# mchitten/keto

Hardware: AMD Instinct MI355X
Metric: permission checks/sec (batched, whole node) + traversal HBM GB/s vs roofline (higher is better)
Workload: dtype u32 ids / u64 bitmasks (integer)

## Files before the change

### keto_amd/csrc/device_engine.hip

```cpp
#include <hip/hip_runtime.h>

#include <algorithm>
#include <atomic>
#include <chrono>
#include <cstring>
#include <functional>
#include <map>
#include <mutex>
#include <string>
#include <thread>
#include <type_traits>
#include <vector>

#include "core_index.hpp"
#include "device_util.hpp"
#include "labels.hpp"
#include "tier.hpp"
#include "ketogpu_internal.hpp"

using namespace ketogpu;
using namespace kdev;

namespace {

// ... 2215 lines not shown
    for (uint32_t step = 32; step; step >>= 1)
        if (step <= (uint32_t)E && pos + step <= (uint32_t)E && L[pos + step - 1] < x) pos += step;
    return pos;
}
template <int E>
__device__ __forceinline__ bool label_find_e(const uint32_t *L, uint32_t x) {
    const uint32_t pos = label_lower_e<E>(L, x);
    return pos < (uint32_t)E && L[pos] == x;
}

template <int E>
__device__ __forceinline__ bool label_block8(const uint32_t *L, uint32_t x) {
    static_assert(E % 8 == 4, "a head's inline entries");
    constexpr int NB = (E + 7) / 8;
    uint32_t blk = 0;
#pragma unroll
    for (int b = 0; b + 1 < NB; b++) blk += L[8 * b + 7] < x;
    const uint4 u = *reinterpret_cast<const uint4 *>(L + 8 * blk);
    const bool lo = min(min(u.x ^ x, u.y ^ x), min(u.z ^ x, u.w ^ x)) == 0;
    if constexpr (NB == 1) {
        return lo;
    } else {
        const uint4 v = *reinterpret_cast<const uint4 *>(L + 8 * blk + 4);
        const bool hi = min(min(v.x ^ x, v.y ^ x), min(v.z ^ x, v.w ^ x)) == 0;
        return lo | (hi & (blk != (uint32_t)(NB - 1)));
    }
}

template <int E, int H>
__device__ __forceinline__ bool label_lookup(const uint32_t *row, uint32_t x) {
    return label_block8<E>(row + kHeadFixed, x);
}

#ifndef KETO_LABEL_MEET
#define KETO_LABEL_MEET 0
#endif

template <int HS, int HP, bool TAIL = false>
__device__ __forceinline__ void label_unit(LabelShared<HS, HP> &sh, const LabelGraph &L, uint32_t r_lane,
                                           uint32_t t_lane, uint64_t *allowed, const uint64_t unit,
                                           const LabelRest &R, const LabelRest &F, unsigned long long *stats) {
    static_assert((HS == 8 || HS == 16 || HS == 32 || HS == 64) && (HP == 8 || HP == 16 || HP == 32 || HP == 64),
                  "heads of 8, 16, 32 or 64 words");
    constexpr int SW = HS / 4, PW = HP / 4;
    constexpr uint32_t CS = HS - kHeadFixed, CP = HP - kHeadFixed;
    const uint32_t lane = threadIdx.x & 63, q = lane >> 2, sub = lane & 3;
    const uint32_t r = (uint32_t)__shfl((int)r_lane, (int)q, 64), t = (uint32_t)__shfl((int)t_lane, (int)q, 64);
    const bool some = r != KETOGPU_NODE_NONE && t != KETOGPU_NODE_NONE;
    const bool valid = some && r < kDynBase;
    uint32_t sw[SW], pw[PW];
#pragma unroll
    for (int k = 0; k < SW; k++) sw[k] = 0xFFFFFFFFu;
#pragma unroll
    for (int k = 0; k < PW; k++) pw[k] = 0xFFFFFFFFu;
    if (valid) {
        label_head_load<SW>(L.S + (uint64_t)t * HS, sub, sw);
        label_head_load<PW>(L.P + (uint64_t)r * HP, sub, pw);
    }
    const uint32_t ns = label_word<SW, 0>(sw), np = label_word<PW, 0>(pw);
    const bool labelled = valid && ns != kNoLabel && np != kNoLabel;
    const uint64_t smask = (uint64_t)label_word<SW, 2>(sw) | (uint64_t)label_word<SW, 3>(sw) << 32;
    const uint64_t pmask = (uint64_t)label_word<PW, 2>(pw) | (uint64_t)label_word<PW, 3>(pw) << 32;
    uint32_t *Sl = sh.S + q * (HS + 4), *Pl = sh.P + q * (HP + 4);
    label_to_lds<SW>(Sl, sw, sub);
    label_to_lds<PW>(Pl, pw, sub);
    const uint32_t *Se = Sl + kHeadFixed, *Pe = Pl + kHeadFixed;
    const uint32_t shard = (uint32_t)(unit % kRestShards);
    {
        const bool rest = sub == 0 && some && !labelled;
        const uint32_t at = lds_append(rest, R.count + shard * kRestStride);
        if (rest) R.list[shard * R.cap + at] = (uint32_t)(unit * 16 + q);
// ... 5 lines not shown
#pragma unroll
    for (int k = 0; k < SW; k++) es += (k >= (int)kHeadFixed || s_body) && sw[k] < L.ni;
    es += (uint32_t)__builtin_amdgcn_update_dpp(0, (int)es, 0xB1, 0xf, 0xf, false);
    es += (uint32_t)__builtin_amdgcn_update_dpp(0, (int)es, 0x4E, 0xf, 0xf, false);
    if (!labelled) es = 0;
    const uint32_t ep = min(np, CP);
    {
        bool head = false, body = false;
#pragma unroll
        for (int k = 0; k < SW; k++) (k < (int)kHeadFixed ? head : body) |= sw[k] == r;
        hit |= labelled && r >= L.ni && (body | (head & s_body));
    }
    if (labelled && !hit) {
        if (KETO_LABEL_MEET == 2) {
            if (es <= ep)
                for (uint32_t k = sub; k < es && !hit; k += 4) hit = label_find_e<CP>(Pe, Se[k]);
            else
                for (uint32_t k = sub; k < ep && !hit; k += 4) hit = label_find_e<CS>(Se, Pe[k]);
        } else {
            if constexpr (HS == HP) {
                const bool ws = es <= ep;
                const uint32_t *W = ws ? Se : Pe, *O = ws ? Pl : Sl;
                const uint32_t e = ws ? es : ep;
                for (uint32_t k = sub; k < e && !hit; k += 4) hit = label_lookup<CP, HP>(O, W[k]);
            } else {
                if (es <= ep)
                    for (uint32_t k = sub; k < es && !hit; k += 4) hit = label_lookup<CP, HP>(Pl, Se[k]);
                else
                    for (uint32_t k = sub; k < ep && !hit; k += 4) hit = label_lookup<CS, HS>(Sl, Pe[k]);
            }
        }
    }
    bool tail = false;
    if constexpr (TAIL) {
        const uint64_t hq = __ballot(hit);
        bool tq = labelled && !((hq >> (lane & ~3u)) & 0xF) && np > CP && np <= 2 * CP && es > 0;
        uint32_t p_last = 0;
        if (tq) {
            const uint32_t s_end = Se[CS - 1];
            p_last = Pe[CP - 1];
            const bool s_whole = ns <= CS || s_end >= L.ni, raw_done = r < L.ni || ns <= CS || r <= s_end;
            tq = s_whole && raw_done && Se[es - 1] > p_last;
        }
        if (__ballot(tq)) {
            uint32_t k0 = 0;
#pragma unroll
            for (int k = 0; k < SW; k++) k0 += (k >= (int)kHeadFixed || s_body) && sw[k] <= p_last;
            k0 += (uint32_t)__builtin_amdgcn_update_dpp(0, (int)k0, 0xB1, 0xf, 0xf, false);
            k0 += (uint32_t)__builtin_amdgcn_update_dpp(0, (int)k0, 0x4E, 0xf, 0xf, false);
            constexpr int NT = (int)CP / 4, NL = (NT + 3) / 4;
            const uint4 *Tg = reinterpret_cast<const uint4 *>(L.P + (uint64_t)label_word<PW, 1>(pw) * 16) + CP / 4;
            uint4 tv[NL];
#pragma unroll
            for (int j = 0; j < NL; j++) {
                const uint32_t i = sub + 4 * j;
                tv[j] = make_uint4(0xFFFFFFFFu, 0xFFFFFFFFu, 0xFFFFFFFFu, 0xFFFFFFFFu);
                if (tq && i < (uint32_t)NT && CP + 4 * i < np) tv[j] = Tg[i];
            }
            wave_sync();
#pragma unroll
            for (int j = 0; j < NL; j++) {
                const uint32_t i = sub + 4 * j, w = CP + 4 * i;
                if (tq && i < (uint32_t)NT)
                    reinterpret_cast<uint4 *>(Pl)[1 + i] =
                        make_uint4(w < np ? tv[j].x : 0xFFFFFFFFu, w + 1 < np ? tv[j].y : 0xFFFFFFFFu,
                                   w + 2 < np ? tv[j].z : 0xFFFFFFFFu, w + 3 < np ? tv[j].w : 0xFFFFFFFFu);
            }
            wave_sync();
            if (tq)
                for (uint32_t k = k0 + sub; k < es && !hit; k += 4) hit = label_lookup<CP, HP>(Pl, Se[k]);
            tail = tq;
        }
    }
    {
        const uint64_t hb = __ballot(hit);
        const uint32_t os = label_word<SW, 1>(sw), op = label_word<PW, 1>(pw);
        bool full = false;
        if (sub == 0 && labelled && !tail && !((hb >> lane) & 0xF)) {
            const uint32_t s_end = Se[CS - 1];
            const bool s_whole = ns <= CS || s_end >= L.ni, p_whole = np <= CP;
            const uint32_t s_last = es ? Se[es - 1] : 0u, p_last = ep ? Pe[ep - 1] : 0u;
            const bool lm_done = es == 0 || np == 0 || (s_whole && (p_whole || s_last <= p_last)) ||
                                 (p_whole && p_last <= s_last);
            const bool raw_done = r < L.ni || ns <= CS || r <= s_end;
            full = !(lm_done && raw_done);
        }
        const uint32_t at = lds_append(full, F.count + shard * kRestStride);
        if (full) {
            uint4 *rec = F.rec + 2 * (shard * F.cap + at);
            rec[0] = make_uint4((uint32_t)(unit * 16 + q), r, t, ns);
            rec[1] = make_uint4(np, os, op, 0u);
        }
    }
    const uint64_t bits = __ballot(hit);
    uint32_t rows = 0, ent = 0;
    if (stats) {
        rows = wave_sum_all(labelled && sub == 0 ? 2u : 0u);
        ent = wave_sum_all(labelled && sub == 0 ? ns + np + kHeadFixed : 0u);
    }
    uint64_t x = bits | bits >> 1;
    x = (x | x >> 2) & 0x1111111111111111ull;
    x = (x | x >> 3) & 0x0303030303030303ull;
    x = (x | x >> 6) & 0x000F000F000F000Full;
    x = (x | x >> 12) & 0x000000FF000000FFull;
    x = (x | x >> 24) & 0xFFFFull;
    if (lane == 0) {
        reinterpret_cast<uint16_t *>(allowed)[unit] = (uint16_t)x;
        if (stats) {
            atomicAdd(&stat_slot(stats)[0], (unsigned long long)rows);
            atomicAdd(&stat_slot(stats)[2], (unsigned long long)ent);
        }
    }
}

__device__ __forceinline__ void label_clear_next(const LabelRest &R, const LabelRest &F) {
    if (blockIdx.x == 0 && threadIdx.x < 64) {
        R.next_count[threadIdx.x * kRestStride] = 0u;
        F.next_count[threadIdx.x * kRestStride] = 0u;
    }
}

template <int HS, int HP>
__global__ __launch_bounds__(64) void label_kernel(LabelGraph L, const uint32_t *roots, const uint32_t *targets,
                                                   uint64_t n, uint64_t *allowed, LabelRest R, LabelRest F,
                                                   unsigned long long *stats, uint64_t unit0) {
    __shared__ LabelShared<HS, HP> sh;
    if (unit0 == 0) label_clear_next(R, F);
    const uint64_t units = (n + 15) / 16;
    const uint64_t unit = unit0 + blockIdx.x;
    uint32_t r, t;
    bidi_load_rt<16>(unit, units, roots, targets, n, r, t);
    label_unit<HS, HP>(sh, L, r, t, allowed, unit, R, F, stats);
    if (unit + 1 == units && threadIdx.x == 0)
        for (uint64_t u = units; u < (units + 3) / 4 * 4; u++) reinterpret_cast<uint16_t *>(allowed)[u] = 0;
}

template <int HS, int HP>
__global__ __launch_bounds__(256) void label_host_kernel(DevGraph g, LabelGraph L, const uint32_t *hr,
                                                         const uint32_t *ht, uint32_t *dr, uint32_t *dt, uint64_t n,
                                                         uint64_t *allowed, LabelRest R, LabelRest F,
                                                         unsigned long long *stats, unsigned long long *first_bad) {
    __shared__ LabelShared<HS, HP> sh[4];
    __shared__ uint32_t rq[2][64];
    const uint32_t wave = threadIdx.x >> 6, lane = threadIdx.x & 63;
    label_clear_next(R, F);
    if (wave == 0) {
        uint32_t r[4], t[4];
        host_unit_requests<4>(g, hr, ht, dr, dt, n, first_bad, r, t);
        if (lane < 16)
#pragma unroll
            for (int k = 0; k < 4; k++) rq[0][16 * k + lane] = r[k], rq[1][16 * k + lane] = t[k];
    }
    __syncthreads();
    const uint64_t units = (n + 15) / 16;
    const uint64_t unit = (uint64_t)blockIdx.x * 4 + wave;
    if (unit >= units) return;
    const uint32_t rk = lane < 16 ? rq[0][16 * wave + lane] : KETOGPU_NODE_NONE;
    const uint32_t tk = lane < 16 ? rq[1][16 * wave + lane] : KETOGPU_NODE_NONE;
    label_unit<HS, HP>(sh[wave], L, rk, tk, allowed, unit, R, F, stats);
}

__device__ __forceinline__ void packed24_decode(uint32_t *raw, const uint64_t *src, uint64_t w0, uint64_t nwords,
                                                uint32_t lane, uint32_t &r, uint32_t &t) {
    if (lane < 48) {
        const uint64_t w = w0 + lane < nwords ? src[w0 + lane] : 0ull;
        *reinterpret_cast<uint2 *>(raw + 2 * lane) = make_uint2((uint32_t)w, (uint32_t)(w >> 32));
    }
    wave_sync();
    const uint32_t k = (3 * lane) >> 1;
    const uint64_t v = ((uint64_t)raw[k + 1] << 32 | raw[k]) >> ((lane & 1) * 16);
    r = (uint32_t)v & 0xFFFFFFu;
    t = (uint32_t)(v >> 24) & 0xFFFFFFu;
    if (r == 0xFFFFFFu) r = KETOGPU_NODE_NONE;
    if (t == 0xFFFFFFu) t = KETOGPU_NODE_NONE;
}

template <int HS, int HP>
__global__ __launch_bounds__(256) void label_host_packed_kernel(DevGraph g, LabelGraph L, const uint64_t *hp,
                                                                uint32_t *dr, uint32_t *dt, uint64_t n,
                                                                uint64_t *allowed, LabelRest R, LabelRest F,
                                                                unsigned long long *stats,
                                                                unsigned long long *first_bad) {
    __shared__ LabelShared<HS, HP> sh[4];
    __shared__ uint32_t rq[2][64];
    const uint32_t wave = threadIdx.x >> 6, lane = threadIdx.x & 63;
    label_clear_next(R, F);
    if (wave == 0) {
        uint32_t r, t;
        packed24_decode(&rq[0][0], hp, (uint64_t)blockIdx.x * 48, (6 * n + 7) / 8, lane, r, t);
        const uint64_t c = (uint64_t)blockIdx.x * 64 + lane;
        if (c < n) {
            if ((r != KETOGPU_NODE_NONE && r >= g.Nx) || (t != KETOGPU_NODE_NONE && t >= g.N)) {
                atomicMin(first_bad, (unsigned long long)c);
                r = t = KETOGPU_NODE_NONE;
            }
            dr[c] = r;
            dt[c] = t;
        } else {
            r = t = KETOGPU_NODE_NONE;
        }
        wave_sync();
        rq[0][lane] = r;
        rq[1][lane] = t;
    }
    __syncthreads();
    const uint64_t units = (n + 15) / 16;
    const uint64_t unit = (uint64_t)blockIdx.x * 4 + wave;
    if (unit >= units) return;
    const uint32_t rk = lane < 16 ? rq[0][16 * wave + lane] : KETOGPU_NODE_NONE;
    const uint32_t tk = lane < 16 ? rq[1][16 * wave + lane] : KETOGPU_NODE_NONE;
    label_unit<HS, HP>(sh[wave], L, rk, tk, allowed, unit, R, F, stats);
}

__host__ __device__ constexpr uint32_t full_stage(int HS, int HP) { return HS >= 64 || HP >= 64 ? 256u : 128u; }

template <int HS, int HP, uint32_t kStage, int kPre, int kFly>
__device__ __forceinline__ uint64_t label_dense_units(uint32_t *stage, const LabelGraph &L, uint64_t *allowed,
                                                      const LabelRest &F, const uint32_t c, const uint32_t first_u,
                                                      const uint32_t stride) {
    static_assert(kStage % 4 == 0, "16-byte aligned rows");
    const uint32_t lane = threadIdx.x, q = lane >> 2, sub = lane & 3;
    const uint32_t nu = (c + 15) / 16;
    const uint32_t incl = wave_incl_sum_u32(nu);
    const uint64_t units = (uint64_t)__builtin_amdgcn_readlane((int)incl, 63);
    uint32_t *row = stage + q * kStage;
    uint64_t ent = 0;
    for (uint64_t u = first_u; u < units; u += stride) {
        const uint32_t shard = (uint32_t)__builtin_ctzll(__ballot(incl > u));
        const uint32_t first = (uint32_t)__builtin_amdgcn_readlane((int)(incl - nu), (int)shard);
        const uint32_t cs = (uint32_t)__builtin_amdgcn_readlane((int)c, (int)shard);
        const uint64_t j = (u - first) * 16 + (lane & 15);
        uint4 r0 = make_uint4(KETOGPU_NODE_NONE, 0, 0, 0), r1 = make_uint4(0, 0, 0, 0);
        if (lane < 16 && j < cs) {
            const uint4 *rec = F.rec + 2 * (shard * F.cap + j);
            r0 = rec[0];
            r1 = rec[1];
        }
        const uint32_t idx = (uint32_t)__shfl((int)r0.x, (int)q, 64);
        const uint32_t rr = (uint32_t)__shfl((int)r0.y, (int)q, 64), tt = (uint32_t)__shfl((int)r0.z, (int)q, 64);
        const uint32_t ns = (uint32_t)__shfl((int)r0.w, (int)q, 64), np = (uint32_t)__shfl((int)r1.x, (int)q, 64);
        const uint32_t os = (uint32_t)__shfl((int)r1.y, (int)q, 64), op = (uint32_t)__shfl((int)r1.z, (int)q, 64);
        const bool valid = idx != KETOGPU_NODE_NONE;
        const bool s_over = ns > (uint32_t)(HS - kHeadFixed), p_over = np > (uint32_t)(HP - kHeadFixed);
        const uint32_t *Sg = s_over ? L.S + (uint64_t)os * 16 : L.S + (uint64_t)tt * HS + kHeadFixed;
        const uint32_t *Pg = p_over ? L.P + (uint64_t)op * 16 : L.P + (uint64_t)rr * HP + kHeadFixed;
        const bool walk_p = np <= ns;
        const uint32_t nw = walk_p ? np : ns, nl = walk_p ? ns : np;
        const uint32_t *Lg = walk_p ? Sg : Pg, *W = walk_p ? Pg : Sg;
        {
            constexpr int kSt = (kStage / 4 + 3) / 4;
            const bool st = valid && nl <= kStage;
#pragma unroll
            for (int k0 = 0; k0 < kSt; k0 += kFly) {
                uint4 v[kFly];
#pragma unroll
                for (int k = 0; k < kFly; k++) {
                    const uint32_t i = sub + 4 * (k0 + k);
                    v[k] = k0 + k < kSt && st && i * 4 < nl ? reinterpret_cast<const uint4 *>(Lg)[i]
                                                            : make_uint4(0u, 0u, 0u, 0u);
                }
#pragma unroll
                for (int k = 0; k < kFly; k++) {
                    const uint32_t i = sub + 4 * (k0 + k);
                    if (k0 + k < kSt && st && i * 4 < nl) reinterpret_cast<uint4 *>(row)[i] = v[k];
                }
            }
        }
        uint32_t wk[kPre];
#pragma unroll
        for (int i = 0; i < kPre; i++) {
            const uint32_t k = sub + 4 * i;
            wk[i] = valid && k < nw ? W[k] : 0u;
        }
        wave_sync();
        const uint32_t *O = nl <= kStage ? row : Lg;
        bool hit = false;
        if (valid) {
#pragma unroll
            for (int i = 0; i < kPre; i++)
                if (!hit && sub + 4 * i < nw) hit = label_find_n(O, nl, wk[i]);
            for (uint32_t k = sub + 4 * kPre; k < nw && !hit; k += 4) hit = label_find_n(O, nl, W[k]);
            if (sub == 0 && !hit && rr >= L.ni) hit = walk_p ? label_find_n(O, nl, rr) : label_find_n(W, nw, rr);
        }
        const uint64_t bits = __ballot(hit);
        if (valid && sub == 0) {
            if ((bits >> lane) & 0xF) atomicOr((unsigned long long *)&allowed[idx >> 6], 1ull << (idx & 63));
            ent += nl;
        }
        wave_sync();
    }
    return ent;
}

template <int HS, int HP>
__global__ __launch_bounds__(64) void label_full_kernel(LabelGraph L, uint64_t *allowed, LabelRest R, LabelRest F,
                                                        unsigned int *total_rest, unsigned int *total_full,
                                                        unsigned long long *stats, unsigned long long *mirror) {
    constexpr uint32_t kFullStage = full_stage(HS, HP);
    __shared__ alignas(16) uint32_t stage[16 * kFullStage];
    const uint32_t lane = threadIdx.x;
    const uint32_t c = F.count[lane * kRestStride];
    if (blockIdx.x == 0) {
        const uint32_t tr = wave_sum_all(R.count[lane * kRestStride]), tf = wave_sum_all(c);
        if (lane == 0) *total_rest = tr, *total_full = tf;
        if (mirror && lane < 12)
            mirror[lane] = lane == 8 ? (unsigned long long)tr : lane == 11 ? (unsigned long long)tf << 32 : 0ull;
    }
    const uint64_t ent =
        label_dense_units<HS, HP, kFullStage, 16, (int)kFullStage / 16>(stage, L, allowed, F, c, blockIdx.x, gridDim.x);
    const uint32_t e = wave_sum_all((uint32_t)ent);
    if (stats && lane == 0 && e) atomicAdd(&stat_slot(stats)[2], (unsigned long long)e);
}

template <int HS, int HP, bool TAIL>
__global__ __launch_bounds__(64) void label_carry_kernel(LabelGraph L, const uint32_t *roots, const uint32_t *targets,
                                                         uint64_t n, uint64_t *allowed, LabelRest R, LabelRest F,
                                                         LabelRest Fd, uint64_t *allowed_d, uint32_t D) {
    __shared__ LabelShared<HS, HP> sh;
    static_assert(sizeof(LabelShared<HS, HP>) == 64 * (HS + HP + 8), "the dense role's stage");
    if (blockIdx.x < D) {
        label_dense_units<HS, HP, HS + HP + 8, 4, 2>(reinterpret_cast<uint32_t *>(&sh), L, allowed_d, Fd,
                                                     Fd.count[threadIdx.x * kRestStride], blockIdx.x, D);
        return;
    }
    if (blockIdx.x == D) {
        R.next_count[threadIdx.x * kRestStride] = 0u;
        F.next_count[threadIdx.x * kRestStride] = 0u;
    }
    const uint64_t units = (n + 15) / 16;
    const uint64_t unit = blockIdx.x - D;
    uint32_t r, t;
    bidi_load_rt<16>(unit, units, roots, targets, n, r, t);
    label_unit<HS, HP, TAIL>(sh, L, r, t, allowed, unit, R, F, nullptr);
    if (unit + 1 == units && threadIdx.x == 0)
        for (uint64_t u = units; u < (units + 3) / 4 * 4; u++) reinterpret_cast<uint16_t *>(allowed)[u] = 0;
}

template <class SH>
__global__ __launch_bounds__(64) void label_rest_kernel(DevGraph g, const FRec *frec, const FRec *brec,
                                                        const uint32_t *roots, const uint32_t *targets,
                                                        uint64_t *allowed, LabelRest R, unsigned int *total,
                                                        uint32_t *out, unsigned int *out_count,
                                                        unsigned long long *stats) {
    __shared__ SH S;
    const uint32_t lane = threadIdx.x;
    const uint32_t c = R.count[lane * kRestStride];
    const uint32_t nu = (c + 15) / 16;
    const uint32_t incl = wave_incl_sum_u32(nu);
    const uint64_t units = (uint64_t)__builtin_amdgcn_readlane((int)incl, 63);
    const uint32_t listed = wave_sum_all(c);
    if (blockIdx.x == 0 && lane == 0) *total = listed;
    for (uint64_t u = blockIdx.x; u < units; u += gridDim.x) {
        const uint32_t shard = (uint32_t)__builtin_ctzll(__ballot(incl > u));
        const uint32_t first = (uint32_t)__builtin_amdgcn_readlane((int)(incl - nu), (int)shard);
        const uint32_t cs = (uint32_t)__builtin_amdgcn_readlane((int)c, (int)shard);
        const uint64_t j = (u - first) * 16 + lane;
        uint32_t idx = KETOGPU_NODE_NONE, r = KETOGPU_NODE_NONE, t = KETOGPU_NODE_NONE;
        if (lane < 16 && j < cs) {
            idx = R.list[shard * R.cap + j];
            r = roots[idx];
            t = targets[idx];
        }
        lite_unit<SH, false>(S, g, frec, brec, bidi_load_rows(g, r, t), allowed, u, out, out_count, stats, nullptr,
                             idx, true);
        __syncthreads();
    }
// ... 1437 lines not shown
    }();
    bool label_clean = false;
    bool lean_call = false;
    bool pipelined_req = false, queued = false;
    hipStream_t pipe_s[kPipe] = {};
    bool pipe_used[kPipe] = {};
    const ketogpu_queries *pipe_q[kPipe] = {};
    bool label_defer = [] {
        const char *e = getenv("KETOGPU_LABEL_DEFER");
        return !e || atoi(e) != 0;
    }();
    int done_mode = [] {
        const char *e = getenv("KETOGPU_LABEL_DONE_EVENT");
        return !e ? 2 : !strcmp(e, "record") ? 0 : !strcmp(e, "nofence") ? 1 : 2;
    }();
    struct PendingDense {
        bool on = false;
        ketogpu_queries *q = nullptr;
        uint64_t *allowed = nullptr;
        LabelRest R{}, F{};
    } pend[kPipe];
    bool carry_call = false;
    unsigned cur_pipe = 0;
    uint64_t pipe_epoch = 1;
    hipEvent_t order_ev = nullptr;
    hipStream_t pstream(unsigned k) const {
        if (k == cur_pipe) return stream;
        return k ? pipe_s[k] : pipe_s[cur_pipe];
    }
    bool label_tail = [] {
        const char *e = getenv("KETOGPU_LABEL_TAIL");
        return !e || atoi(e) != 0;
    }();
    uint64_t piped_full = 0;
    bool piped_full_known = false, flush_unread = false;
    void take_piped_full() {
        piped_full = ((const unsigned int *)(h_ctr + 24))[7];
        piped_full_known = true;
    }
    static unsigned grid_for(uint64_t full) { return (unsigned)std::min<uint64_t>(std::max<uint64_t>(full / 16 + 64, 64), 16384); }
    unsigned dense_grid() const { return grid_for(full_prev); }
    unsigned piped_grid() const { return grid_for(piped_full_known ? piped_full : full_prev); }
    bool flush_dense(unsigned k) {
        PendingDense p = pend[k];
        if (!p.on) return false;
        pend[k] = PendingDense{};
        label_dispatch([&](auto hs, auto hp) {
            KLAUNCH((label_full_kernel<decltype(hs)::value, decltype(hp)::value>), dim3(piped_grid()), dim3(64), 0,
                    pstream(k), lgraph, p.allowed, p.R, p.F, &spill_count[0], &spill_count[7], nullptr, d_hctr + 16);
        });
        flush_unread = true;
        if (p.q) {
            if (p.q->done_ev) HIP_CHECK(hipEventRecord(p.q->done_ev, pstream(k)));
            p.q->pass = 0;
        }
        return true;
    }
    void flush_dense_all() {
        for (unsigned k = 0; k < kPipe; k++) flush_dense(k);
    }
    void drain_pipe() {
        flush_dense_all();
        for (unsigned k = 0; k < kPipe; k++) {
            pipe_q[k] = nullptr;
            if (pipe_used[k]) HIP_CHECK(hipStreamSynchronize(pstream(k)));
            pipe_used[k] = false;
// ... 9 lines not shown
    }
    uint64_t label_nolabel_heads = 0;
    bool plan_auto = false;
    double label_overflow_share[2] = {0, 0};
    uint32_t label_knob = 0;
    bool label_rest_free(const Batch &q) const {
        return use_label && label_nolabel_heads == 0 && label_knob == 0 && lab_invalid == 0 && !q.has_dyn;
    }
    uint64_t full_prev = 1024 * 16;
    uint32_t label_hs = 16, label_hp = 8;
    double label_coverage = 0, label_build_ms = 0, label_pll_ms = 0;
    uint64_t label_bytes = 0, label_entries = 0;
    uint64_t label_nwords[2] = {0, 0};
    std::shared_ptr<const ReachLabels> lab_R;
    std::vector<uint32_t> lab_cap[2], lab_ovf[2];
    std::vector<uint64_t> lab_succ;
    std::vector<uint8_t> lab_pinv;
    uint64_t lab_invalid = 0, lab_rewritten = 0, lab_relabels = 0;
    uint32_t lab_permille = 0;
    template <class F>
    void label_dispatch(F &&f) {
        auto hp = [&](auto hs) {
            if (label_hp == 8) f(hs, std::integral_constant<int, 8>{});
            else if (label_hp == 16) f(hs, std::integral_constant<int, 16>{});
            else if (label_hp == 32) f(hs, std::integral_constant<int, 32>{});
            else f(hs, std::integral_constant<int, 64>{});
        };
        if (label_hs == 8) hp(std::integral_constant<int, 8>{});
        else if (label_hs == 16) hp(std::integral_constant<int, 16>{});
        else if (label_hs == 32) hp(std::integral_constant<int, 32>{});
        else hp(std::integral_constant<int, 64>{});
    }
    void launch_label_host(const Batch &q, const HostSrc *src, uint64_t bunits) {
        if (src->packed) {
            label_dispatch([&](auto hs, auto hp) {
                KLAUNCH((label_host_packed_kernel<decltype(hs)::value, decltype(hp)::value>),
                        dim3((unsigned)((bunits + 3) / 4)), dim3(256), 0, stream, g, lgraph,
                        (const uint64_t *)src->packed, io->d_roots, io->d_targets, q.n, q.allowed, label_rest(q.n),
                        label_full(q.n), st.stats, d_bad);
            });
            return;
        }
        label_dispatch([&](auto hs, auto hp) {
            KLAUNCH((label_host_kernel<decltype(hs)::value, decltype(hp)::value>), dim3((unsigned)((bunits + 3) / 4)),
                    dim3(256), 0, stream, g, lgraph, src->roots, src->targets, io->d_roots, io->d_targets, q.n,
                    q.allowed, label_rest(q.n), label_full(q.n), st.stats, d_bad);
        });
    }
    int core_shape = 2;
    uint64_t closure_nodes[2] = {0, 0}, closure_entries[2] = {0, 0};
    double core_build_ms = 0;
    DevGraph gcore() const {
        DevGraph x = g;
        for (int d = 0; d < 2; d++) {
            x.blk[d] = core_blk[d];
            x.blk_log[d] = core_blk_log[d];
        }
        return x;
    }
    bool frec_needed = false;
    static constexpr uint64_t kTrialMin = 1 << 16;
    static constexpr int kTrialRuns = 2;
    int trials_left = 0;
    struct Candidate {
        bool bidi;
        int hlog, bt, f, lf;
        double ms;
        bool units = true;
        int u = 16;
        int wpe = 1;
        int lite = 0;
    };
    std::vector<Candidate> candidates;
    struct BidiCfg {
        int hlog, bt, f, lf;
        int u = 16;
        int wpe = 1;
        int lite = 0;
        bool operator==(const BidiCfg &o) const {
            return hlog == o.hlog && bt == o.bt && f == o.f && lf == o.lf && u == o.u && wpe == o.wpe &&
                   lite == o.lite;
        }
    };
    BidiCfg bidi_cfg{9, 64, KETO_F1, 7};

    void launch_bidi(const BidiCfg &c, unsigned grid, unsigned pad, const Batch &q, const uint32_t *parents,
                     const unsigned int *in_count, uint32_t *out, unsigned int *out_count, unsigned long long *stats,
                     unsigned long long *stp, uint64_t unit0 = 0, hipStream_t stream = nullptr, bool chunked = false) {
        if (!stream) stream = this->stream;
        if (c.lite == 3) {
            label_dispatch([&](auto hs, auto hp) {
                KLAUNCH((label_kernel<decltype(hs)::value, decltype(hp)::value>), dim3(grid), dim3(64), pad, stream,
                        lgraph, q.roots, q.targets, q.n, q.allowed, label_rest(q.n), label_full(q.n), stats, unit0);
            });
            return;
        }
        if (c.lite == 2) {
#define KETO_CORE_K(SH)                                                                                       \
    KLAUNCH((lite_kernel<SH, true>), dim3(grid), dim3(64), pad, stream, gcore(), core_rec[0], core_rec[1], q.roots, \
            q.targets, q.n, q.allowed, out, out_count, stats, unit0, stp)
            if (core_shape == 1)
                KETO_CORE_K(CoreShapeS);
            else if (core_shape == 2)
                KETO_CORE_K(CoreShapeM);
            else
                KETO_CORE_K(LiteShape);
#undef KETO_CORE_K
            return;
        }
        if (c.lite) {
            if (c.u == 32)
                KLAUNCH((lite_kernel<LiteShape32>), dim3(grid), dim3(64), pad, stream, g, frec, brec, q.roots,
                        q.targets, q.n, q.allowed, out, out_count, stats, unit0, stp);
            else
                KLAUNCH((lite_kernel<LiteShape>), dim3(grid), dim3(64), pad, stream, g, frec, brec, q.roots, q.targets,
                        q.n, q.allowed, out, out_count, stats, unit0, stp);
            return;
        }
        if (chunked && c == BidiCfg{9, 64, KETO_F1, 7, 16, 1}) {
            KLAUNCH((bidi_kernel<16, 9, KETO_F1, 64, 7, 1, 1>), dim3(grid), dim3(64), pad, stream, g, frec, brec, q.roots,
                    q.targets, q.n, q.allowed, parents, in_count, 1u, out, out_count, stats, stp, unit0);
            return;
        }
#define KETO_BIDI_U(U, HL, F, BT, LF, WPE)                                                                        \
    if (c == BidiCfg{HL, BT, F, LF, U, WPE}) {                                                                   \
        KLAUNCH((bidi_kernel<U, HL, F, BT, LF, WPE>), dim3(grid), dim3(BT), pad, stream, g, frec, brec,          \
// ... 1086 lines not shown
    }

    uint32_t read_spill_count() {
        HIP_CHECK(hipMemcpyAsync(h_ctr + 12, spill_count, sizeof(unsigned int), hipMemcpyDeviceToHost, stream));
        HIP_CHECK(hipStreamSynchronize(stream));
        return (uint32_t)h_ctr[12];
    }

    uint64_t bidi_tail(const Batch &q, ketogpu_run_stats &rs, std::vector<std::pair<hipEvent_t, hipEvent_t>> &unit_ev,
                       hipEvent_t a, hipEvent_t b, uint64_t bunits, const std::function<void()> &before_sync = {}) {
        uint32_t *list[2] = {spill_units, spill_units + spill_cap};
        hipEvent_t d = ev();
        std::vector<SpillStage> stages;
        for (const SpillStage &sg : cascade)
            if (sg.u <= (stages.empty() ? bidi_cfg.u : stages.back().u)) stages.push_back(sg);
        int u_prev = bidi_cfg.u;
        std::vector<uint32_t> fans;
        for (const SpillStage &sg : stages) {
            fans.push_back((uint32_t)(u_prev / sg.u));
            u_prev = sg.u;
        }
        if (bidi_cfg.lite == 3) {
            stages.assign(1, SpillStage{1, 'L'});
            fans.assign(1, 1u);
            u_prev = 1;
        }
        const int cur = (int)(stages.size() & 1);
        static const bool eager_env = getenv("KETOGPU_CASCADE_EAGER") != nullptr;
        const bool lazy = !eager_env && !cascade_log && stage_prev[0] == 0;
        const EmitReq E = emit_req;
        emit_req = EmitReq{};
        const bool fused = bidi_cfg.lite == 3 && lean_call;
        if (fused && (!lazy || E.out)) throw Error(KETOGPU_EDEVICE, "lean label call without a lazy rest stage");
        if (bidi_cfg.lite == 3 && !carry_call)
            label_dispatch([&](auto hs, auto hp) {
                KLAUNCH((label_full_kernel<decltype(hs)::value, decltype(hp)::value>), dim3(dense_grid()), dim3(64), 0,
                        stream, lgraph, q.allowed, label_rest(q.n), label_full(q.n), &spill_count[0], &spill_count[7],
                        fused ? nullptr : st.stats + 4 * kStatSlots, fused ? d_hctr + 16 : nullptr);
            });
        if (carry_call) {
            PendingDense &p = pend[cur_pipe];
            p.on = true;
            p.q = nullptr;
            p.allowed = q.allowed;
            p.R = label_rest(q.n);
            p.F = label_full(q.n);
        }
        if (fused && pipelined_req && !trials_left && label_rest_free(q)) {
            queued = true;
            unit_end = d;
            rs.rest_requests = 0;
            rs.full_requests = full_prev;
            label_clean = true;
            label_calls++;
            rs.push_launches += carry_call ? 1 : 2;
            rs.unit_launches += carry_call ? 1 : 2;
            return 0;
        }
        auto launch_stages = [&](uint64_t prev0) {
            for (size_t k = 0, c = 0; k < stages.size(); k++, c ^= 1)
                launch_stage(stages[k], q, list[c], &spill_count[k], fans[k], list[c ^ 1], &spill_count[k + 1],
                             st.stats + 4 * kStatSlots, k == 0 ? prev0 : k < 8 ? stage_prev[k] : ~0ull);
        };
        if (!lazy) launch_stages(stage_prev[0]);
        if (b) HIP_CHECK(hipEventRecord(d, stream));
        const size_t ns = stages.size() + 1;
        static_assert(kStatsLen == 8 + 8 * kStatSlots + 12, "statistics layout");
        const unsigned eb = E.out ? (unsigned)std::min<uint64_t>(blocks_for(2 * E.words + 1), 255) : 0;
        if (!fused)
            KLAUNCH(stats_reduce_kernel, dim3(1 + eb), dim3(kBlock), 0, stream, st.stats + 8, 2, stat_out(), d_hctr + 16,
                    12, E);
        if (before_sync) before_sync();
        if (!b && !lean_call) HIP_CHECK(hipEventRecord(d, stream));
        wait_stream();
        const unsigned int *cnt = (const unsigned int *)(h_ctr + 24);
        size_t launched = lazy ? 1 : stages.size() + 1;
        if (lazy && cnt[0]) {
            d = ev();
            launch_stages((uint64_t)cnt[0] * fans[0]);
            KLAUNCH(stats_reduce_kernel, dim3(1 + eb), dim3(kBlock), 0, stream, st.stats + 8, 2, stat_out(),
                    d_hctr + 16, 12, E);
            if (before_sync) before_sync();
            if (!lean_call) HIP_CHECK(hipEventRecord(d, stream));
            wait_stream();
            launched = stages.size() + 2;
        }
        unit_end = d;
        if (b) {
            unit_ev.push_back({a, b});
            unit_ev.push_back({b, d});
        } else if (!lean_call) {
            unit_ev.push_back({a, d});
        }
        const uint64_t *t = (const uint64_t *)h_ctr + 16;
        rs.main_bytes = 16 * t[0] + 16 * t[1] + 4 * t[2] + 8 * q.n + 8 * ((q.n + 63) / 64);
        if (cascade_log) {
            fprintf(stderr, "[cascade] units %llu, spills per stage:", (unsigned long long)bunits);
            for (size_t k = 0; k < ns; k++) fprintf(stderr, " %u", cnt[k]);
            fprintf(stderr, "\n");
        }
        for (size_t k = 0; k < ns; k++) rs.spilled_units += cnt[k];
        if (bidi_cfg.lite == 3) {
            rs.rest_requests = cnt[0];
            rs.full_requests = cnt[7];
            full_prev = cnt[7];
            label_clean = fused && cnt[0] == 0;
        }
        for (size_t k = 0; k < stages.size() && k < 8; k++) stage_prev[k] = (uint64_t)cnt[k] * fans[k];
        rs.push_launches += launched;
// ... 47 lines not shown
                                   q.roots, q.targets, q.n, q.allowed, q.flags, list[0], spill_count, st.stats);
            HIP_CHECK(hipEventRecord(b, stream));
            unit_ev.push_back({a, b});
            uint64_t left = read_spill_count();
            rs.spilled_units += left;
            rs.push_launches++;
            if (!left) return 0;
            HIP_CHECK(hipMemsetAsync(spill_count, 0, sizeof(unsigned int), stream));
            a = ev();
            b = ev();
            HIP_CHECK(hipEventRecord(a, stream));
            KLAUNCH(unit_kernel<1>, dim3((unsigned)(left * wave_u)), dim3(kBlock), 0, stream, g, has_kids,
                               q.roots, q.targets, q.n, q.allowed, q.flags, list[0], (uint32_t)wave_u, list[1],
                               spill_count, st.stats, nullptr);
            HIP_CHECK(hipEventRecord(b, stream));
            unit_ev.push_back({a, b});
            left = read_spill_count();
            rs.spilled_units += left;
            rs.push_launches++;
            if (left)
                HIP_CHECK(hipMemcpyAsync(list[0], list[1], left * sizeof(uint32_t), hipMemcpyDeviceToDevice, stream));
            return left;
        }
        uint64_t units = (q.n + 15) / 16;
        uint64_t left = 0;
        if (use_v2 || (use_lite && use_bidi)) {
            if (use_bidi) {
                const bool direct = src && src->mapped && pipe_direct &&
                                    (bidi_cfg == BidiCfg{9, 64, KETO_F1, 7, 16, 1} || bidi_cfg.lite);
                const bool light = light_begin && (direct || !src);
                hipEvent_t a = light ? light_begin : ev(), b = light ? nullptr : ev();
                if (!light) HIP_CHECK(hipEventRecord(a, stream));
                const uint64_t bunits = (q.n + bidi_cfg.u - 1) / bidi_cfg.u;
                if (!src && carry_call) {
                    PendingDense p = pend[cur_pipe];
                    pend[cur_pipe] = PendingDense{};
                    const unsigned D = p.on ? piped_grid() : 0u;
                    label_dispatch([&](auto hs, auto hp) {
                        if (label_tail)
                            KLAUNCH((label_carry_kernel<decltype(hs)::value, decltype(hp)::value, true>),
                                    dim3(D + (unsigned)bunits), dim3(64), lds_pad, stream, lgraph, q.roots, q.targets,
                                    q.n, q.allowed, label_rest(q.n), label_full(q.n), p.F, p.allowed, D);
                        else
                            KLAUNCH((label_carry_kernel<decltype(hs)::value, decltype(hp)::value, false>),
                                    dim3(D + (unsigned)bunits), dim3(64), lds_pad, stream, lgraph, q.roots, q.targets,
                                    q.n, q.allowed, label_rest(q.n), label_full(q.n), p.F, p.allowed, D);
                    });
                    if (p.q) p.q->pass = 2;
                } else if (!src) {
                    launch_bidi(bidi_cfg, (unsigned)bunits, lds_pad, q, nullptr, nullptr, list[0], &spill_count[0],
                                lean_call ? nullptr : st.stats, stamps);
                } else if (direct) {
#define KETO_HOST_K(K)                                                                                     \
    do {                                                                                                   \
        if (bidi_cfg.lite == 3)                                                                            \
            launch_label_host(q, src, bunits);                                                             \
        else if (bidi_cfg.lite == 2 && core_shape == 1)                                                    \
            KLAUNCH((lite_host_kernel<K, CoreShapeS, true>), dim3((unsigned)((bunits + K - 1) / K)), dim3(64), \
                    0, stream, gcore(), core_rec[0], core_rec[1], src->roots, src->targets, io->d_roots,   \
                    io->d_targets, q.n, q.allowed, list[0], &spill_count[0], st.stats, d_bad);              \
        else if (bidi_cfg.lite == 2 && core_shape == 2)                                                    \
            KLAUNCH((lite_host_kernel<K, CoreShapeM, true>), dim3((unsigned)((bunits + K - 1) / K)), dim3(64), \
                    0, stream, gcore(), core_rec[0], core_rec[1], src->roots, src->targets, io->d_roots,   \
                    io->d_targets, q.n, q.allowed, list[0], &spill_count[0], st.stats, d_bad);              \
        else if (bidi_cfg.lite == 2)                                                                       \
            KLAUNCH((lite_host_kernel<K, LiteShape, true>), dim3((unsigned)((bunits + K - 1) / K)), dim3(64), \
// ... 315 lines not shown
                  : use_v2    ? 2
                              : 4;
        rs.plan_lists = use_units && !wave_u && use_bidi ? (uint32_t)bidi_cfg.f : 0;
        rs.plan_unit = use_units && !wave_u && use_bidi ? (uint32_t)bidi_cfg.u : 0;
        rs.hubs = n_hubs;
        rs.hub_words = hub_words;
        rs.hub_build_ms = hub_build_ms;
        rs.closure_cap_f = use_core ? closure_cap[0] : 0;
        rs.closure_cap_b = use_core ? closure_cap[1] : 0;
        rs.closure_nodes_f = closure_nodes[0];
        rs.closure_nodes_b = closure_nodes[1];
        rs.closure_entries_f = closure_entries[0];
        rs.closure_entries_b = closure_entries[1];
        rs.core_build_ms = core_build_ms;
        rs.label_on = use_label ? 1 : 0;
        rs.label_s_head = use_label ? label_hs : 0;
        rs.label_p_head = use_label ? label_hp : 0;
        rs.label_coverage = label_coverage;
        rs.label_build_ms = label_build_ms;
        rs.label_pll_ms = label_pll_ms;
        rs.label_bytes = label_bytes;
        rs.label_entries = label_entries;
        rs.label_rewritten = lab_rewritten;
        rs.label_marked = lab_invalid;
        rs.label_relabels = lab_relabels;
        ev_used = 0;
        std::vector<std::pair<hipEvent_t, hipEvent_t>> push_ev, pull_ev;
        hipEvent_t t_begin = ev(), t_end = ev();
        uint64_t words = (q.n + 63) / 64;
        const bool label_resident = !src && use_units && !wave_u && use_bidi && bidi_cfg.lite == 3 && q.n;
        static const bool eager_env = getenv("KETOGPU_CASCADE_EAGER") != nullptr;
        lean_call = label_resident && fuse_reduce && light_events && !eager_env && !cascade_log && stage_prev[0] == 0;
        carry_call = lean_call && label_defer && pipelined_req && !trials_left && label_rest_free(q);
        if (!carry_call)
            flush_dense_all();
        else if (pend[cur_pipe].on && pend[cur_pipe].allowed == q.allowed)
            flush_dense(cur_pipe);
        const auto h0 = std::chrono::steady_clock::now();
        light_begin = nullptr;
        if (light_events && (src || (use_units && !wave_u && use_bidi && q.n && bidi_cfg.lite == 3))) {
            if (!lean_call) HIP_CHECK(hipEventRecord(t_begin, stream));
            light_begin = t_begin;
        }
        const bool skip_clear = lean_call && label_clean && qq.flags_zero && !clear_bad;
        label_clean = false;
        qq.flags_zero = false;
        if (!skip_clear)
            KLAUNCH(clear_kernel, dim3(64), dim3(kBlock), 0, stream, q.allowed, std::max<uint64_t>(words, 1),
                    q.flags, std::max<uint64_t>(words, 1), st.stats, (uint64_t)kStatsLen, clear_bad);
        clear_bad = nullptr;
        const bool bidi_first = use_units && !wave_u && (use_v2 || use_lite) && use_bidi && q.n;
        if (!bidi_first && !light_begin) HIP_CHECK(hipEventRecord(t_begin, stream));
        std::vector<std::pair<hipEvent_t, hipEvent_t>> unit_ev;
        if (use_units && q.n) {
            uint64_t ns = run_units(q, rs, unit_ev, src, before_sync);
            if (bidi_first && !lean_call) {
                if (!unit_ev.empty())
                    t_begin = unit_ev.front().first;
                else
                    HIP_CHECK(hipEventRecord(t_begin, stream));
            }
            rs.spilled_requests = ns;
            if (ns) {
                KLAUNCH(spill_gather_kernel, dim3(blocks_for(ns)), dim3(kBlock), 0, stream, spill_units, ns,
                                   q.roots, q.targets, q.n, spill_roots, spill_targets);
                Batch sb = q;
// ... 662 lines not shown
```

Measured before the change: 24.72 billion.

## Settle overflow label checks inline in the label kernel instead of a separate dense pass

```diff
diff --git a/keto_amd/csrc/device_engine.hip b/keto_amd/csrc/device_engine.hip
--- a/keto_amd/csrc/device_engine.hip
+++ b/keto_amd/csrc/device_engine.hip
@@ -2271,11 +2271,63 @@
     return label_block8<E>(row + kHeadFixed, x);
 }
 
+template <int HS, int HP, uint32_t kStage, int kPre, int kFly>
+__device__ __forceinline__ bool label_dense_request(uint32_t *row, const LabelGraph &L, const bool valid,
+                                                    const uint32_t sub, const uint32_t rr, const uint32_t tt,
+                                                    const uint32_t ns, const uint32_t np, const uint32_t os,
+                                                    const uint32_t op, uint32_t &nl_out) {
+    static_assert(kStage % 4 == 0, "16-byte aligned rows");
+    const bool s_over = ns > (uint32_t)(HS - kHeadFixed), p_over = np > (uint32_t)(HP - kHeadFixed);
+    const uint32_t *Sg = s_over ? L.S + (uint64_t)os * 16 : L.S + (uint64_t)tt * HS + kHeadFixed;
+    const uint32_t *Pg = p_over ? L.P + (uint64_t)op * 16 : L.P + (uint64_t)rr * HP + kHeadFixed;
+    const bool walk_p = np <= ns;
+    const uint32_t nw = walk_p ? np : ns, nl = walk_p ? ns : np;
+    const uint32_t *Lg = walk_p ? Sg : Pg, *W = walk_p ? Pg : Sg;
+    nl_out = nl;
+    {
+        constexpr int kSt = (kStage / 4 + 3) / 4;
+        const bool st = valid && nl <= kStage;
+#pragma unroll
+        for (int k0 = 0; k0 < kSt; k0 += kFly) {
+            uint4 v[kFly];
+#pragma unroll
+            for (int k = 0; k < kFly; k++) {
+                const uint32_t i = sub + 4 * (k0 + k);
+                v[k] = k0 + k < kSt && st && i * 4 < nl ? reinterpret_cast<const uint4 *>(Lg)[i]
+                                                        : make_uint4(0u, 0u, 0u, 0u);
+            }
+#pragma unroll
+            for (int k = 0; k < kFly; k++) {
+                const uint32_t i = sub + 4 * (k0 + k);
+                if (k0 + k < kSt && st && i * 4 < nl) reinterpret_cast<uint4 *>(row)[i] = v[k];
+            }
+        }
+    }
+    uint32_t wk[kPre];
+#pragma unroll
+    for (int i = 0; i < kPre; i++) {
+        const uint32_t k = sub + 4 * i;
+        wk[i] = valid && k < nw ? W[k] : 0u;
+    }
+    wave_sync();
+    const uint32_t *O = nl <= kStage ? row : Lg;
+    bool hit = false;
+    if (valid) {
+#pragma unroll
+        for (int i = 0; i < kPre; i++)
+            if (!hit && sub + 4 * i < nw) hit = label_find_n(O, nl, wk[i]);
+        for (uint32_t k = sub + 4 * kPre; k < nw && !hit; k += 4) hit = label_find_n(O, nl, W[k]);
+        if (sub == 0 && !hit && rr >= L.ni) hit = walk_p ? label_find_n(O, nl, rr) : label_find_n(W, nw, rr);
+    }
+    return hit;
+}
+
 #ifndef KETO_LABEL_MEET
 #define KETO_LABEL_MEET 0
 #endif
 
-template <int HS, int HP, bool TAIL = false>
+constexpr int kLabelPlain = 0, kLabelTail = 1, kLabelSettle = 2;
+template <int HS, int HP, int MODE = kLabelPlain>
 __device__ __forceinline__ void label_unit(LabelShared<HS, HP> &sh, const LabelGraph &L, uint32_t r_lane,
                                            uint32_t t_lane, uint64_t *allowed, const uint64_t unit,
                                            const LabelRest &R, const LabelRest &F, unsigned long long *stats) {
@@ -2347,7 +2399,7 @@
         }
     }
     bool tail = false;
-    if constexpr (TAIL) {
+    if constexpr (MODE != kLabelPlain) {
         const uint64_t hq = __ballot(hit);
         bool tq = labelled && !((hq >> (lane & ~3u)) & 0xF) && np > CP && np <= 2 * CP && es > 0;
         uint32_t p_last = 0;
@@ -2387,6 +2439,7 @@
             tail = tq;
         }
     }
+    bool open = false;
     {
         const uint64_t hb = __ballot(hit);
         const uint32_t os = label_word<SW, 1>(sw), op = label_word<PW, 1>(pw);
@@ -2400,18 +2453,31 @@
             const bool raw_done = r < L.ni || ns <= CS || r <= s_end;
             full = !(lm_done && raw_done);
         }
-        const uint32_t at = lds_append(full, F.count + shard * kRestStride);
-        if (full) {
-            uint4 *rec = F.rec + 2 * (shard * F.cap + at);
-            rec[0] = make_uint4((uint32_t)(unit * 16 + q), r, t, ns);
-            rec[1] = make_uint4(np, os, op, 0u);
+        if constexpr (MODE == kLabelSettle) {
+            open = sub == 0 && (full || tail);
+            lds_append(open, F.count + shard * kRestStride);
+            const uint64_t fb = __ballot(full);
+            if (fb) {
+                wave_sync();
+                uint32_t nl;
+                hit |= label_dense_request<HS, HP, HS + HP + 8, 4, 2>(
+                    reinterpret_cast<uint32_t *>(&sh) + q * (HS + HP + 8), L, ((fb >> (lane & ~3u)) & 1) != 0, sub, r, t,
+                    ns, np, os, op, nl);
+            }
+        } else {
+            const uint32_t at = lds_append(full, F.count + shard * kRestStride);
+            if (full) {
+                uint4 *rec = F.rec + 2 * (shard * F.cap + at);
+                rec[0] = make_uint4((uint32_t)(unit * 16 + q), r, t, ns);
+                rec[1] = make_uint4(np, os, op, 0u);
+            }
         }
     }
     const uint64_t bits = __ballot(hit);
     uint32_t rows = 0, ent = 0;
     if (stats) {
         rows = wave_sum_all(labelled && sub == 0 ? 2u : 0u);
-        ent = wave_sum_all(labelled && sub == 0 ? ns + np + kHeadFixed : 0u);
+        ent = wave_sum_all(labelled && sub == 0 ? ns + np + kHeadFixed + (open ? max(ns, np) : 0u) : 0u);
     }
     uint64_t x = bits | bits >> 1;
     x = (x | x >> 2) & 0x1111111111111111ull;
@@ -2435,7 +2501,7 @@
     }
 }
 
-template <int HS, int HP>
+template <int HS, int HP, int MODE = kLabelPlain>
 __global__ __launch_bounds__(64) void label_kernel(LabelGraph L, const uint32_t *roots, const uint32_t *targets,
                                                    uint64_t n, uint64_t *allowed, LabelRest R, LabelRest F,
                                                    unsigned long long *stats, uint64_t unit0) {
@@ -2445,12 +2511,12 @@
     const uint64_t unit = unit0 + blockIdx.x;
     uint32_t r, t;
     bidi_load_rt<16>(unit, units, roots, targets, n, r, t);
-    label_unit<HS, HP>(sh, L, r, t, allowed, unit, R, F, stats);
+    label_unit<HS, HP, MODE>(sh, L, r, t, allowed, unit, R, F, stats);
     if (unit + 1 == units && threadIdx.x == 0)
         for (uint64_t u = units; u < (units + 3) / 4 * 4; u++) reinterpret_cast<uint16_t *>(allowed)[u] = 0;
 }
 
-template <int HS, int HP>
+template <int HS, int HP, int MODE = kLabelPlain>
 __global__ __launch_bounds__(256) void label_host_kernel(DevGraph g, LabelGraph L, const uint32_t *hr,
                                                          const uint32_t *ht, uint32_t *dr, uint32_t *dt, uint64_t n,
                                                          uint64_t *allowed, LabelRest R, LabelRest F,
@@ -2472,7 +2538,7 @@
     if (unit >= units) return;
     const uint32_t rk = lane < 16 ? rq[0][16 * wave + lane] : KETOGPU_NODE_NONE;
     const uint32_t tk = lane < 16 ? rq[1][16 * wave + lane] : KETOGPU_NODE_NONE;
-    label_unit<HS, HP>(sh[wave], L, rk, tk, allowed, unit, R, F, stats);
+    label_unit<HS, HP, MODE>(sh[wave], L, rk, tk, allowed, unit, R, F, stats);
 }
 
 __device__ __forceinline__ void packed24_decode(uint32_t *raw, const uint64_t *src, uint64_t w0, uint64_t nwords,
@@ -2490,7 +2556,7 @@
     if (t == 0xFFFFFFu) t = KETOGPU_NODE_NONE;
 }
 
-template <int HS, int HP>
+template <int HS, int HP, int MODE = kLabelPlain>
 __global__ __launch_bounds__(256) void label_host_packed_kernel(DevGraph g, LabelGraph L, const uint64_t *hp,
                                                                 uint32_t *dr, uint32_t *dt, uint64_t n,
                                                                 uint64_t *allowed, LabelRest R, LabelRest F,
@@ -2524,7 +2590,7 @@
     if (unit >= units) return;
     const uint32_t rk = lane < 16 ? rq[0][16 * wave + lane] : KETOGPU_NODE_NONE;
     const uint32_t tk = lane < 16 ? rq[1][16 * wave + lane] : KETOGPU_NODE_NONE;
-    label_unit<HS, HP>(sh[wave], L, rk, tk, allowed, unit, R, F, stats);
+    label_unit<HS, HP, MODE>(sh[wave], L, rk, tk, allowed, unit, R, F, stats);
 }
 
 __host__ __device__ constexpr uint32_t full_stage(int HS, int HP) { return HS >= 64 || HP >= 64 ? 256u : 128u; }
@@ -2533,7 +2599,6 @@
 __device__ __forceinline__ uint64_t label_dense_units(uint32_t *stage, const LabelGraph &L, uint64_t *allowed,
                                                       const LabelRest &F, const uint32_t c, const uint32_t first_u,
                                                       const uint32_t stride) {
-    static_assert(kStage % 4 == 0, "16-byte aligned rows");
     const uint32_t lane = threadIdx.x, q = lane >> 2, sub = lane & 3;
     const uint32_t nu = (c + 15) / 16;
     const uint32_t incl = wave_incl_sum_u32(nu);
@@ -2556,47 +2621,8 @@
         const uint32_t ns = (uint32_t)__shfl((int)r0.w, (int)q, 64), np = (uint32_t)__shfl((int)r1.x, (int)q, 64);
         const uint32_t os = (uint32_t)__shfl((int)r1.y, (int)q, 64), op = (uint32_t)__shfl((int)r1.z, (int)q, 64);
         const bool valid = idx != KETOGPU_NODE_NONE;
-        const bool s_over = ns > (uint32_t)(HS - kHeadFixed), p_over = np > (uint32_t)(HP - kHeadFixed);
-        const uint32_t *Sg = s_over ? L.S + (uint64_t)os * 16 : L.S + (uint64_t)tt * HS + kHeadFixed;
-        const uint32_t *Pg = p_over ? L.P + (uint64_t)op * 16 : L.P + (uint64_t)rr * HP + kHeadFixed;
-        const bool walk_p = np <= ns;
-        const uint32_t nw = walk_p ? np : ns, nl = walk_p ? ns : np;
-        const uint32_t *Lg = walk_p ? Sg : Pg, *W = walk_p ? Pg : Sg;
-        {
-            constexpr int kSt = (kStage / 4 + 3) / 4;
-            const bool st = valid && nl <= kStage;
-#pragma unroll
-            for (int k0 = 0; k0 < kSt; k0 += kFly) {
-                uint4 v[kFly];
-#pragma unroll
-                for (int k = 0; k < kFly; k++) {
-                    const uint32_t i = sub + 4 * (k0 + k);
-                    v[k] = k0 + k < kSt && st && i * 4 < nl ? reinterpret_cast<const uint4 *>(Lg)[i]
-                                                            : make_uint4(0u, 0u, 0u, 0u);
-                }
-#pragma unroll
-                for (int k = 0; k < kFly; k++) {
-                    const uint32_t i = sub + 4 * (k0 + k);
-                    if (k0 + k < kSt && st && i * 4 < nl) reinterpret_cast<uint4 *>(row)[i] = v[k];
-                }
-            }
-        }
-        uint32_t wk[kPre];
-#pragma unroll
-        for (int i = 0; i < kPre; i++) {
-            const uint32_t k = sub + 4 * i;
-            wk[i] = valid && k < nw ? W[k] : 0u;
-        }
-        wave_sync();
-        const uint32_t *O = nl <= kStage ? row : Lg;
-        bool hit = false;
-        if (valid) {
-#pragma unroll
-            for (int i = 0; i < kPre; i++)
-                if (!hit && sub + 4 * i < nw) hit = label_find_n(O, nl, wk[i]);
-            for (uint32_t k = sub + 4 * kPre; k < nw && !hit; k += 4) hit = label_find_n(O, nl, W[k]);
-            if (sub == 0 && !hit && rr >= L.ni) hit = walk_p ? label_find_n(O, nl, rr) : label_find_n(W, nw, rr);
-        }
+        uint32_t nl;
+        const bool hit = label_dense_request<HS, HP, kStage, kPre, kFly>(row, L, valid, sub, rr, tt, ns, np, os, op, nl);
         const uint64_t bits = __ballot(hit);
         if (valid && sub == 0) {
             if ((bits >> lane) & 0xF) atomicOr((unsigned long long *)&allowed[idx >> 6], 1ull << (idx & 63));
@@ -2605,6 +2631,20 @@
         wave_sync();
     }
     return ent;
+}
+
+__device__ __forceinline__ void label_totals(const LabelRest &R, const uint32_t c, unsigned int *total_rest,
+                                             unsigned int *total_full, unsigned long long *mirror) {
+    const uint32_t lane = threadIdx.x;
+    const uint32_t tr = wave_sum_all(R.count[lane * kRestStride]), tf = wave_sum_all(c);
+    if (lane == 0) *total_rest = tr, *total_full = tf;
+    if (mirror && lane < 12)
+        mirror[lane] = lane == 8 ? (unsigned long long)tr : lane == 11 ? (unsigned long long)tf << 32 : 0ull;
+}
+
+__global__ __launch_bounds__(64) void label_totals_kernel(LabelRest R, LabelRest F, unsigned int *total_rest,
+                                                          unsigned int *total_full, unsigned long long *mirror) {
+    label_totals(R, F.count[threadIdx.x * kRestStride], total_rest, total_full, mirror);
 }
 
 template <int HS, int HP>
@@ -2615,12 +2655,7 @@
     __shared__ alignas(16) uint32_t stage[16 * kFullStage];
     const uint32_t lane = threadIdx.x;
     const uint32_t c = F.count[lane * kRestStride];
-    if (blockIdx.x == 0) {
-        const uint32_t tr = wave_sum_all(R.count[lane * kRestStride]), tf = wave_sum_all(c);
-        if (lane == 0) *total_rest = tr, *total_full = tf;
-        if (mirror && lane < 12)
-            mirror[lane] = lane == 8 ? (unsigned long long)tr : lane == 11 ? (unsigned long long)tf << 32 : 0ull;
-    }
+    if (blockIdx.x == 0) label_totals(R, c, total_rest, total_full, mirror);
     const uint64_t ent =
         label_dense_units<HS, HP, kFullStage, 16, (int)kFullStage / 16>(stage, L, allowed, F, c, blockIdx.x, gridDim.x);
     const uint32_t e = wave_sum_all((uint32_t)ent);
@@ -2646,7 +2681,7 @@
     const uint64_t unit = blockIdx.x - D;
     uint32_t r, t;
     bidi_load_rt<16>(unit, units, roots, targets, n, r, t);
-    label_unit<HS, HP, TAIL>(sh, L, r, t, allowed, unit, R, F, nullptr);
+    label_unit<HS, HP, TAIL ? kLabelTail : kLabelPlain>(sh, L, r, t, allowed, unit, R, F, nullptr);
     if (unit + 1 == units && threadIdx.x == 0)
         for (uint64_t u = units; u < (units + 3) / 4 * 4; u++) reinterpret_cast<uint16_t *>(allowed)[u] = 0;
 }
@@ -4150,6 +4185,11 @@
         const char *e = getenv("KETOGPU_LABEL_TAIL");
         return !e || atoi(e) != 0;
     }();
+    bool label_settle = [] {
+        const char *e = getenv("KETOGPU_LABEL_SETTLE");
+        return !e || atoi(e) != 0;
+    }();
+    bool settle_call = false;
     uint64_t piped_full = 0;
     bool piped_full_known = false, flush_unread = false;
     void take_piped_full() {
@@ -4225,9 +4265,16 @@
         else hp(std::integral_constant<int, 64>{});
     }
     void launch_label_host(const Batch &q, const HostSrc *src, uint64_t bunits) {
+        if (settle_call)
+            launch_label_host_mode<kLabelSettle>(q, src, bunits);
+        else
+            launch_label_host_mode<kLabelPlain>(q, src, bunits);
+    }
+    template <int MODE>
+    void launch_label_host_mode(const Batch &q, const HostSrc *src, uint64_t bunits) {
         if (src->packed) {
             label_dispatch([&](auto hs, auto hp) {
-                KLAUNCH((label_host_packed_kernel<decltype(hs)::value, decltype(hp)::value>),
+                KLAUNCH((label_host_packed_kernel<decltype(hs)::value, decltype(hp)::value, MODE>),
                         dim3((unsigned)((bunits + 3) / 4)), dim3(256), 0, stream, g, lgraph,
                         (const uint64_t *)src->packed, io->d_roots, io->d_targets, q.n, q.allowed, label_rest(q.n),
                         label_full(q.n), st.stats, d_bad);
@@ -4235,9 +4282,9 @@
             return;
         }
         label_dispatch([&](auto hs, auto hp) {
-            KLAUNCH((label_host_kernel<decltype(hs)::value, decltype(hp)::value>), dim3((unsigned)((bunits + 3) / 4)),
-                    dim3(256), 0, stream, g, lgraph, src->roots, src->targets, io->d_roots, io->d_targets, q.n,
-                    q.allowed, label_rest(q.n), label_full(q.n), st.stats, d_bad);
+            KLAUNCH((label_host_kernel<decltype(hs)::value, decltype(hp)::value, MODE>),
+                    dim3((unsigned)((bunits + 3) / 4)), dim3(256), 0, stream, g, lgraph, src->roots, src->targets,
+                    io->d_roots, io->d_targets, q.n, q.allowed, label_rest(q.n), label_full(q.n), st.stats, d_bad);
         });
     }
     int core_shape = 2;
@@ -4283,8 +4330,13 @@
         if (!stream) stream = this->stream;
         if (c.lite == 3) {
             label_dispatch([&](auto hs, auto hp) {
-                KLAUNCH((label_kernel<decltype(hs)::value, decltype(hp)::value>), dim3(grid), dim3(64), pad, stream,
-                        lgraph, q.roots, q.targets, q.n, q.allowed, label_rest(q.n), label_full(q.n), stats, unit0);
+                if (settle_call && !chunked)
+                    KLAUNCH((label_kernel<decltype(hs)::value, decltype(hp)::value, kLabelSettle>), dim3(grid),
+                            dim3(64), pad, stream, lgraph, q.roots, q.targets, q.n, q.allowed, label_rest(q.n),
+                            label_full(q.n), stats, unit0);
+                else
+                    KLAUNCH((label_kernel<decltype(hs)::value, decltype(hp)::value>), dim3(grid), dim3(64), pad, stream,
+                            lgraph, q.roots, q.targets, q.n, q.allowed, label_rest(q.n), label_full(q.n), stats, unit0);
             });
             return;
         }
@@ -5437,7 +5489,10 @@
         emit_req = EmitReq{};
         const bool fused = bidi_cfg.lite == 3 && lean_call;
         if (fused && (!lazy || E.out)) throw Error(KETOGPU_EDEVICE, "lean label call without a lazy rest stage");
-        if (bidi_cfg.lite == 3 && !carry_call)
+        if (bidi_cfg.lite == 3 && settle_call)
+            KLAUNCH(label_totals_kernel, dim3(1), dim3(64), 0, stream, label_rest(q.n), label_full(q.n), &spill_count[0],
+                    &spill_count[7], fused ? d_hctr + 16 : nullptr);
+        else if (bidi_cfg.lite == 3 && !carry_call)
             label_dispatch([&](auto hs, auto hp) {
                 KLAUNCH((label_full_kernel<decltype(hs)::value, decltype(hp)::value>), dim3(dense_grid()), dim3(64), 0,
                         stream, lgraph, q.allowed, label_rest(q.n), label_full(q.n), &spill_count[0], &spill_count[7],
@@ -5480,6 +5535,7 @@
         wait_stream();
         const unsigned int *cnt = (const unsigned int *)(h_ctr + 24);
         size_t launched = lazy ? 1 : stages.size() + 1;
+        if (bidi_cfg.lite == 3 && !settle_call) launched++;
         if (lazy && cnt[0]) {
             d = ev();
             launch_stages((uint64_t)cnt[0] * fans[0]);
@@ -5593,6 +5649,8 @@
                 hipEvent_t a = light ? light_begin : ev(), b = light ? nullptr : ev();
                 if (!light) HIP_CHECK(hipEventRecord(a, stream));
                 const uint64_t bunits = (q.n + bidi_cfg.u - 1) / bidi_cfg.u;
+                const bool queued_call = lean_call && pipelined_req && !trials_left && label_rest_free(q);
+                settle_call = label_settle && bidi_cfg.lite == 3 && !b && !queued_call && (!src || direct);
                 if (!src && carry_call) {
                     PendingDense p = pend[cur_pipe];
                     pend[cur_pipe] = PendingDense{};
@@ -5974,6 +6032,7 @@
         static const bool eager_env = getenv("KETOGPU_CASCADE_EAGER") != nullptr;
         lean_call = label_resident && fuse_reduce && light_events && !eager_env && !cascade_log && stage_prev[0] == 0;
         carry_call = lean_call && label_defer && pipelined_req && !trials_left && label_rest_free(q);
+        settle_call = false;
         if (!carry_call)
             flush_dense_all();
         else if (pend[cur_pipe].on && pend[cur_pipe].allowed == q.allowed)
```

Result: slower. 24.44 billion (-1.1%).
